# owensgroup/sparsify.me

Hardware: AMD Instinct MI355X
Metric: effective GF/s (2:4 spmma vs dense gemm) on ResNet-50 layer shapes (higher is better)
Workload: dtype f16

## Files before the change

### sparsify.me_amd/csrc/spmma_f16_fused.hip

```cpp
#include "select24.h"
#include "spmma_args.h"

namespace sm {

constexpr int MAXG = 8;
struct FusedArgs {
  const half_t* A[MAXG];
  const half_t* B[MAXG];
  half_t* C[MAXG];
  size_t sA, sB, sC;
  int Mrows, N, K, lda;
  int batch, tiles_m, tiles_n;
  int ngroup;
  float alpha, beta;
  const half_t* const* dAp;
  const half_t* const* dBp;
  half_t* const* dCp;
};

struct FusedArgsEpi : FusedArgs {
  EpiArgs e;
};
template <bool EPI> struct FusedArgsSel { typedef FusedArgs type; };
template <> struct FusedArgsSel<true> { typedef FusedArgsEpi type; };

template <int BN, int NS, bool BF = false, int BM = 128, int NWV = 4, bool ANT = true, bool DENSE = false, bool EPI = false>
__global__ __launch_bounds__(64 * NWV, (BN == 128 && NWV == 4 && BM == 128) ? 4 : 1) void spmma_f16_fused_direct_kernel(const typename FusedArgsSel<EPI>::type p) {
  static_assert(BM == 128 || BM == 64, "row tile");
  static_assert(NWV == 4 || (NWV == 8 && BM == 128), "waves per workgroup");
  constexpr int NW = NWV, TM = BM / NW, FM = TM / 16, FN = BN / 16;
  constexpr int SA = BM * 128, SB = 64 * BN * 2, STAGE = SA + SB;
  constexpr int A_N = BM / 8, B_N = BN / 8, W = A_N + B_N;
  static_assert(W % NW == 0, "equal DMA share per wave");
  constexpr int SL = W / NW;
  extern __shared__ __attribute__((aligned(16))) char smem[];

  const unsigned tid = threadIdx.x, lane = tid & 63u;
  const unsigned wave = __builtin_amdgcn_readfirstlane(tid >> 6);
  const unsigned tiles = (unsigned)p.tiles_m * (unsigned)p.tiles_n;
  const unsigned lid = tile_order(blockIdx.x, gridDim.x, true);
  const unsigned gb = lid / tiles, trem = lid - gb * tiles;
  const unsigned grp = gb / (unsigned)p.batch, b = gb - grp * (unsigned)p.batch;
  const unsigned tile_m = trem / (unsigned)p.tiles_n, tile_n = trem - tile_m * (unsigned)p.tiles_n;
  const int m0 = (int)tile_m * BM, n0 = (int)tile_n * BN;
  const int nkt = p.K / 64;
  const half_t* A = p.dAp ? p.dAp[gb] : p.A[grp] + (size_t)b * p.sA;
  const half_t* B = p.dBp ? p.dBp[gb] : p.B[grp] + (size_t)b * p.sB;
  half_t* C = p.dCp ? p.dCp[gb] : p.C[grp] + (size_t)b * p.sC;
  const int mlast = p.Mrows - 1;
  EpiBias<FM, FN> eb;
  if constexpr (EPI) eb = epi_bias_prefetch<FM, FN>(p.e, true, wave * TM, 0, m0, n0, p.Mrows, p.N, lane);

  const char* src[SL];
  size_t step[SL];
  unsigned loff[SL];
#pragma unroll
  for (int i = 0; i < SL; ++i) {
    const unsigned t = wave + (unsigned)NW * i;
    if (t < (unsigned)A_N) {
      const unsigned row = 8u * t + (lane >> 3), cs = (lane & 7u) ^ (row & 7u);
      int gr = m0 + (int)row;
      gr = gr < mlast ? gr : mlast;
      src[i] = reinterpret_cast<const char*>(A + (size_t)gr * p.lda) + 16u * cs;
      step[i] = 128;
      loff[i] = t * 1024u;
    } else {
      const unsigned j = t - A_N, panel = j >> 3, kr = 8u * (j & 7u) + (lane >> 3);
      const unsigned cs = (lane & 7u) ^ b_swz(kr);
      int gc = n0 + (int)(64u * panel + 8u * cs);
      gc = gc <= p.N - 8 ? gc : p.N - 8;
      src[i] = reinterpret_cast<const char*>(B + (size_t)kr * p.N + gc);
      step[i] = (size_t)64 * p.N * 2;
      loff[i] = SA + panel * 8192u + (j & 7u) * 1024u;
    }
  }
  auto stage = [&](int kt, int buf) {
    char* base = smem + buf * STAGE;
    static_assert(A_N % NW == 0, "A / B split of the DMA instructions is per instruction index");
#pragma unroll
    for (int i = 0; i < SL; ++i) {
      if (ANT && NW * i < A_N)
        __builtin_amdgcn_global_load_lds((gptr_t*)(src[i] + (size_t)kt * step[i]), (lptr_t*)(base + loff[i]), 16, 0, 2);
      else
        __builtin_amdgcn_global_load_lds((gptr_t*)(src[i] + (size_t)kt * step[i]), (lptr_t*)(base + loff[i]), 16, 0, 0);
    }
  };

  f4 acc[FM][FN];
#pragma unroll
  for (int i = 0; i < FM; ++i)
#pragma unroll
    for (int j = 0; j < FN; ++j) acc[i][j] = f4{0.f, 0.f, 0.f, 0.f};

#pragma unroll
  for (int s = 0; s < NS - 1; ++s)
    if (s < nkt) stage(s, s);
  int cur = 0, fill = NS - 1;
  for (int kt = 0; kt < nkt; ++kt) {
    const int ahead = (nkt - 1 - kt) < (NS - 2) ? (nkt - 1 - kt) : (NS - 2);
    if (NS >= 4 && ahead == 2) wait_dma_and_barrier<2 * SL>();
    else if (NS >= 3 && ahead == 1) wait_dma_and_barrier<SL>();
    else wait_dma_and_barrier<0>();
    if (kt + NS - 1 < nkt) stage(kt + NS - 1, fill);
    const char* As = smem + cur * STAGE;
    if constexpr (DENSE) mfma_stage_dense_a<FM, FN, BF>(As, As + SA, wave * TM, 0, lane, acc);
    else smfmac_stage_dense_a<FM, FN, BF>(As, As + SA, wave * TM, 0, lane, acc);
    cur = cur + 1 == NS ? 0 : cur + 1;
    fill = fill + 1 == NS ? 0 : fill + 1;
  }
  __syncthreads();
  if constexpr (EPI) store_c_tile_epi<BM, BN, FM, FN, 64 * NW, BF>(smem, C, p.e.R + (size_t)b * p.e.sR, p.e, eb, acc, true, wave * TM, 0, m0, n0, p.Mrows, p.N, p.alpha, p.beta, tid);
  else store_c_tile<BM, BN, FM, FN, 64 * NW, BF>(smem, C, acc, true, wave * TM, 0, m0, n0, p.Mrows, p.N, p.alpha, p.beta, tid);
}

template <int BN, int NS, bool BF = false, int BM = 128, int NWV = 4, bool ANT = true, bool DENSE = false, bool EPI = false>
static int launch_fused_direct(const typename FusedArgsSel<EPI>::type& a0, hipStream_t st) {
  typename FusedArgsSel<EPI>::type a = a0;
  a.tiles_m = (a.Mrows + BM - 1) / BM;
  a.tiles_n = (a.N + BN - 1) / BN;
  const size_t nwg = (size_t)a.tiles_m * a.tiles_n * a.batch * a.ngroup;
  constexpr size_t stage_bytes = BM * 128 + 64 * BN * 2;
  const size_t lds_main = ((size_t)(a.K / 64) < (size_t)NS ? (size_t)(a.K / 64) : (size_t)NS) * stage_bytes;
  constexpr size_t lds_epi = (size_t)BM * (BN * 2 + 16);
  const size_t lds = lds_main > lds_epi ? lds_main : lds_epi;
  constexpr size_t lds_max = NS * stage_bytes > lds_epi ? NS * stage_bytes : lds_epi;
  return launch_grid<&spmma_f16_fused_direct_kernel<BN, NS, BF, BM, NWV, ANT, DENSE, EPI>>(nwg, 64 * NWV, lds_max, lds, st, "sm_spmma_fused_f16",
                                                                                          "spmma_f16_fused_direct_kernel", a);
}

template <int BN, bool BF = false, int NSA = 3, int NSB = 2, bool ANT = true, bool DENSE = false, bool EPI = false>
__global__ __launch_bounds__(512) void spmma_f16_fused_big_kernel(const typename FusedArgsSel<EPI>::type p) {
  constexpr int BM = 256, NW = 8, TM = BM / NW, FM = TM / 16, FN = BN / 16;
  constexpr int SA = BM * 128, SB = 64 * BN * 2;
  constexpr int A_N = BM / 8, B_N = BN / 8;
  static_assert(A_N % NW == 0 && B_N % NW == 0, "equal DMA share per wave");
  static_assert(NSA == 3 && (NSB == 2 || NSB == 3), "ring depths the counted waits below are written for");
  constexpr int SLA = A_N / NW, SLB = B_N / NW;
  constexpr int AHEAD = SLA + (NSB == 3 ? SLB : 0);
  constexpr int BRING = NSA * SA;
  extern __shared__ __attribute__((aligned(16))) char smem[];

  const unsigned tid = threadIdx.x, lane = tid & 63u;
  const unsigned wave = __builtin_amdgcn_readfirstlane(tid >> 6);
  const unsigned tiles = (unsigned)p.tiles_m * (unsigned)p.tiles_n;
  const unsigned lid = xcd_remap(blockIdx.x, gridDim.x);
  const unsigned gb = lid / tiles, trem = lid - gb * tiles;
  const unsigned grp = gb / (unsigned)p.batch, b = gb - grp * (unsigned)p.batch;
  const unsigned tile_m = trem / (unsigned)p.tiles_n, tile_n = trem - tile_m * (unsigned)p.tiles_n;
  const int m0 = (int)tile_m * BM, n0 = (int)tile_n * BN;
  const int nkt = p.K / 64;
  const half_t* A = p.dAp ? p.dAp[gb] : p.A[grp] + (size_t)b * p.sA;
  const half_t* B = p.dBp ? p.dBp[gb] : p.B[grp] + (size_t)b * p.sB;
  half_t* C = p.dCp ? p.dCp[gb] : p.C[grp] + (size_t)b * p.sC;
  const int mlast = p.Mrows - 1;
// ... 370 lines not shown
    set_error("%s", why);
    return SM_STATUS_NOT_SUPPORTED;
  }
  SkPlan pl = sk_plan(panels, nkt, (size_t)a.tiles_n, (size_t)cus);
  const size_t nwg = (size_t)pl.slots * a.tiles_n;
  if (!workspace || !aligned16(workspace) || workspace_bytes < sk_workspace_bytes(nwg, BN)) {
    set_error("sm_spmma_fused_*_ws: the stream-K form needs a 16-byte aligned workspace of sm_spmma_fused_workspace_size bytes");
    return SM_STATUS_INVALID_VALUE;
  }
  SkArgs s = {};
  s.flags = reinterpret_cast<unsigned*>(workspace);
  s.part = reinterpret_cast<float*>(reinterpret_cast<char*>(workspace) + 4096);
  s.panels = (unsigned)panels; s.slots = pl.slots; s.tg = pl.tg; s.wg = pl.wg; s.groups_full = pl.groups_full; s.tgl = pl.tgl; s.wgl = pl.wgl;
  for (int i = 0; i < 9; ++i) { s.cut[i] = pl.cut[i]; s.cutl[i] = pl.cutl[i]; }
  constexpr size_t lds_main = (size_t)3 * BM * 128 + (size_t)2 * 64 * BN * 2;
  constexpr size_t lds_epi = (size_t)BM * (BN * 2 + 16);
  constexpr size_t lds = lds_main > lds_epi ? lds_main : lds_epi;
  static_assert(lds > 64 * 1024 && lds <= 160 * 1024, "LDS budget of the stream-K kernel (always opted in)");
  return launch_grid<&spmma_f16_fused_sk_kernel<BN, BF, ANT, DENSE>>(nwg, 512, lds, lds, st, "sm_spmma_fused_f16", "spmma_f16_fused_sk_kernel", a, s);
}

static bool sk_takes(size_t rows, size_t problems, size_t n, size_t k, bool astat_shape, size_t cus, SkPlan& pl) {
  if (n <= 128 || k < 128 || k % 64 != 0) return false;
  const size_t nkt = k / 64;
  const size_t panels = (rows + 255) / 256 * problems, tn = (n + 255) / 256;
  const size_t t_big = panels * tn, t_wide = (rows + 127) / 128 * tn * problems;
  pl = sk_plan(panels, nkt, tn, cus);
  if (!pl.slots) return false;
  const double c_sk = (double)pl.units + (pl.wg > 1 ? 8.0 : 0.0);
  const double c_big = (double)((t_big + cus - 1) / cus * nkt), c_wide = 0.6 * (double)((t_wide + cus - 1) / cus * nkt);
  const double c_now = c_big < c_wide ? c_big : c_wide;
  return !astat_shape && pl.wg > 1 && c_sk < 0.85 * c_now;
}

__device__ __attribute__((aligned(256))) const unsigned char sm_fused_zero_page[256] = {0};

template <int BN, bool BF = false, bool DENSE = false, bool EPI = false>
__global__ __launch_bounds__(256) void spmma_f16_fused_span_kernel(const typename FusedArgsSel<EPI>::type p, const unsigned span_lds ,
                                                                   const size_t a_bytes ) {
  constexpr int BM = 128, NW = 4, TM = BM / NW, FM = TM / 16, FN = BN / 16;
  constexpr int SB = 64 * BN * 2;
  extern __shared__ __attribute__((aligned(16))) char smem[];
  const unsigned tid = threadIdx.x, lane = tid & 63u;
  const unsigned wave = __builtin_amdgcn_readfirstlane(tid >> 6);
  const unsigned tiles = (unsigned)p.tiles_m * (unsigned)p.tiles_n;
  const unsigned lid = xcd_remap(blockIdx.x, gridDim.x);
  const unsigned grp = lid / tiles, trem = lid - grp * tiles;
  const unsigned tile_m = trem / (unsigned)p.tiles_n, tile_n = trem - tile_m * (unsigned)p.tiles_n;
  const int m0 = (int)tile_m * BM, n0 = (int)tile_n * BN;
  const int nkt = (p.K + 63) / 64;
  const char* A = reinterpret_cast<const char*>(p.dAp ? p.dAp[grp] : p.A[grp]);
  const half_t* B = p.dBp ? p.dBp[grp] : p.B[grp];
  half_t* C = p.dCp ? p.dCp[grp] : p.C[grp];
  const unsigned rowbytes = (unsigned)p.K * 2u;
  const int rows = p.Mrows - m0 < BM ? p.Mrows - m0 : BM;
  EpiBias<FM, FN> eb;
  if constexpr (EPI) eb = epi_bias_prefetch<FM, FN>(p.e, true, wave * TM, 0, m0, n0, p.Mrows, p.N, lane);

  {
    const size_t s0 = (size_t)m0 * rowbytes;
    const unsigned len = (unsigned)rows * rowbytes;
    const unsigned np = (len + 1023u) / 1024u;
    const size_t last16 = a_bytes - 16;
    for (unsigned pc = wave; pc < np; pc += NW) {
      size_t off = s0 + (size_t)pc * 1024u + 16u * lane;
      off = off < last16 ? off : last16;
      __builtin_amdgcn_global_load_lds((gptr_t*)(A + off), (lptr_t*)(smem + pc * 1024u), 16, 0, 2);
    }
  }
  char* const Bimg = smem + span_lds;
  {
    constexpr int B_N = BN / 8;
    const int npb = nkt * B_N;
    for (int t = (int)wave; t < npb; t += NW) {
      const int kt = t / B_N, j = t - kt * B_N;
      const unsigned panel = (unsigned)j >> 3, kr = 8u * ((unsigned)j & 7u) + (lane >> 3);
      const unsigned cs = (lane & 7u) ^ b_swz(kr);
      int gc = n0 + (int)(64u * panel + 8u * cs);
      gc = gc <= p.N - 8 ? gc : p.N - 8;
      const int krow = kt * 64 + (int)kr;
      const char* src = krow < p.K ? reinterpret_cast<const char*>(B + (size_t)krow * p.N + gc)
                                   : reinterpret_cast<const char*>(sm_fused_zero_page) + 16u * (lane & 7u);
      __builtin_amdgcn_global_load_lds((gptr_t*)src, (lptr_t*)(Bimg + kt * SB + panel * 8192u + ((unsigned)j & 7u) * 1024u), 16, 0, 0);
    }
  }
  wait_dma_and_barrier<0>();

  f4 acc[FM][FN];
#pragma unroll
  for (int i = 0; i < FM; ++i)
#pragma unroll
    for (int j = 0; j < FN; ++j) acc[i][j] = f4{0.f, 0.f, 0.f, 0.f};
  const unsigned g = lane >> 4, r = lane & 15u;
  unsigned rowoff[FM];
#pragma unroll
  for (int i = 0; i < FM; ++i) {
    int row = (int)(wave * TM + i * 16 + r);
    row = row < rows ? row : rows - 1;
    rowoff[i] = (unsigned)row * rowbytes;
  }
  for (int kt = 0; kt < nkt; ++kt) {
    if constexpr (DENSE) {
      h8 a0[FM], a1[FM];
#pragma unroll
      for (int i = 0; i < FM; ++i) {
        uint32_t d[2][4];
#pragma unroll
        for (int h = 0; h < 2; ++h) {
          const int k0 = kt * 64 + 32 * h + 8 * (int)g;
          int nv = p.K - k0;
          nv = nv < 0 ? 0 : (nv > 8 ? 8 : nv);
          const char* src = smem + rowoff[i] + 2u * (unsigned)k0;
#pragma unroll
          for (int e = 0; e < 4; ++e) {
            const uint32_t lo16 = *reinterpret_cast<const unsigned short*>(src + 4 * e);
            const uint32_t hi16 = *reinterpret_cast<const unsigned short*>(src + 4 * e + 2);
            uint32_t v = lo16 | (hi16 << 16);
            v = 2 * e + 1 < nv ? v : (2 * e < nv ? (v & 0xffffu) : 0u);
            d[h][e] = v;
          }
        }
        a0[i] = __builtin_bit_cast(h8, u4{d[0][0], d[0][1], d[0][2], d[0][3]});
        a1[i] = __builtin_bit_cast(h8, u4{d[1][0], d[1][1], d[1][2], d[1][3]});
      }
      mfma_b_sweep<FM, FN, BF>(a0, a1, Bimg + kt * SB, 0, lane, acc);
      continue;
    }
    h8 af[FM];
    int idx[FM];
    const int k0 = kt * 64 + 16 * (int)g;
    int nv = p.K - k0;
    nv = nv < 0 ? 0 : (nv > 16 ? 16 : nv);
#pragma unroll
    for (int i = 0; i < FM; ++i) {
      const char* src = smem + rowoff[i] + 2u * (unsigned)k0;
      uint32_t d[8];
#pragma unroll
      for (int e = 0; e < 8; ++e) {
        const uint32_t lo16 = *reinterpret_cast<const unsigned short*>(src + 4 * e);
        const uint32_t hi16 = *reinterpret_cast<const unsigned short*>(src + 4 * e + 2);
        uint32_t v = lo16 | (hi16 << 16);
        v = 2 * e + 1 < nv ? v : (2 * e < nv ? (v & 0xffffu) : 0u);
        d[e] = v;
      }
      dense16_to_operand(u4{d[0], d[1], d[2], d[3]}, u4{d[4], d[5], d[6], d[7]}, af[i], idx[i]);
    }
    smfmac_b_sweep<FM, FN, BF>(af, idx, Bimg + kt * SB, 0, lane, acc);
  }
  __syncthreads();
  if constexpr (EPI) store_c_tile_epi<BM, BN, FM, FN, 64 * NW, BF>(smem, C, p.e.R, p.e, eb, acc, true, wave * TM, 0, m0, n0, p.Mrows, p.N, p.alpha, p.beta, tid);
  else store_c_tile<BM, BN, FM, FN, 64 * NW, BF>(smem, C, acc, true, wave * TM, 0, m0, n0, p.Mrows, p.N, p.alpha, p.beta, tid);
}

template <int BN, bool BF = false, bool DENSE = false, bool EPI = false>
static int launch_fused_span(const typename FusedArgsSel<EPI>::type& a0, hipStream_t st) {
  typename FusedArgsSel<EPI>::type a = a0;
  a.tiles_m = (a.Mrows + 127) / 128;
  a.tiles_n = (a.N + BN - 1) / BN;
  const size_t nwg = (size_t)a.tiles_m * a.tiles_n * a.ngroup;
  if (nwg == 0) return SM_STATUS_SUCCESS;
  const size_t kc = ((size_t)a.K + 63) / 64 * 64;
  const size_t span_lds = ((size_t)128 * a.K * 2 + 128 + 1023) / 1024 * 1024;
  const size_t lds_main = span_lds + kc * BN * 2;
  constexpr size_t lds_epi = (size_t)128 * (BN * 2 + 16);
  const size_t lds = lds_main > lds_epi ? lds_main : lds_epi;
  if (lds > 160 * 1024 || nwg > 0x7fffffffu) {
    set_error("sm_spmma_fused_{f16,bf16}: k too long for the span form (use the staged path)");
    return SM_STATUS_NOT_SUPPORTED;
  }
  return launch_grid<&spmma_f16_fused_span_kernel<BN, BF, DENSE, EPI>>(nwg, 256, 160 * 1024, lds, st, "sm_spmma_fused_f16", "spmma_f16_fused_span_kernel", a,
                                                                      (unsigned)span_lds, (size_t)a.Mrows * a.K * 2);
}

template <int BN, int NBW>
struct BTileDma {
  static constexpr int B_WI = (BN / 8) / NBW;
  const char* src[B_WI];
  unsigned dst[B_WI];
  size_t step;
  __device__ __forceinline__ void setup(const half_t* B, int N, int n0, unsigned bw, unsigned lane, unsigned ring_off) {
#pragma unroll
    for (int i = 0; i < B_WI; ++i) {
      const unsigned j = bw + (unsigned)NBW * i, panel = j >> 3, grp = j & 7u, kr = 8u * grp + (lane >> 3);
      const unsigned cs = (lane & 7u) ^ b_swz(kr);
      int gc = n0 + (int)(64u * panel + 8u * cs);
      gc = gc <= N - 8 ? gc : N - 8;
      src[i] = reinterpret_cast<const char*>(B) + ((size_t)kr * N + (size_t)gc) * 2;
      dst[i] = ring_off + panel * 8192u + grp * 1024u;
    }
    step = (size_t)64 * N * 2;
  }
  __device__ __forceinline__ void issue(char* smem, int kt, unsigned buf_off) const {
#pragma unroll
    for (int i = 0; i < B_WI; ++i)
      __builtin_amdgcn_global_load_lds((gptr_t*)(src[i] + (size_t)kt * step), (lptr_t*)(smem + buf_off + dst[i]), 16, 0, 0);
  }
};


template <int BN, int WM, int WN, int NLB, int PF, int NSB, bool BF = false, bool ANT = true, bool EPI = false>
__global__ __launch_bounds__(64 * (WM * WN + 4 + NLB)) void spmma_f16_fused_wide_kernel(const typename FusedArgsSel<EPI>::type p) {
  constexpr int BM = 128, NLA = 4, NC = WM * WN, NW = NC + NLA + NLB;
  static_assert(PF >= 1 && PF <= 3 && NSB >= 2 && NSB <= 4, "pipeline depths");
  constexpr int TM = BM / WM, TN = BN / WN, FM = TM / 16, FN = TN / 16;
  constexpr int SA = BM * 64, SM_ = BM * 8, ASTG = SA + SM_, SB = 64 * BN * 2;
  constexpr int BRING = 2 * ASTG;
  constexpr int NBW = NLB > 0 ? NLB : WM * WN;
  constexpr int B_N = BN / 8, B_WI = B_N / NBW;
  static_assert(B_N % NBW == 0 && B_WI >= 1 && (NSB - 2) * B_WI <= 63, "B tile vs issuing waves");
  extern __shared__ __attribute__((aligned(16))) char smem[];

  const unsigned tid = threadIdx.x, lane = tid & 63u;
  const unsigned wave = __builtin_amdgcn_readfirstlane(tid >> 6);
  const unsigned tiles = (unsigned)p.tiles_m * (unsigned)p.tiles_n;
  const unsigned lid = xcd_remap(blockIdx.x, gridDim.x);
  const unsigned gb = lid / tiles, trem = lid - gb * tiles;
  const unsigned grp = gb / (unsigned)p.batch, b = gb - grp * (unsigned)p.batch;
  const unsigned tile_m = trem / (unsigned)p.tiles_n, tile_n = trem - tile_m * (unsigned)p.tiles_n;
  const int m0 = (int)tile_m * BM, n0 = (int)tile_n * BN;
  const int nkt = p.K / 64;
  half_t* C = p.C[grp] + (size_t)b * p.sC;

  f4 acc[FM][FN];
#pragma unroll
  for (int i = 0; i < FM; ++i)
#pragma unroll
    for (int j = 0; j < FN; ++j) acc[i][j] = f4{0.f, 0.f, 0.f, 0.f};
  const unsigned wm = wave / WN, wn = wave % WN;
  EpiBias<FM, FN> eb;
  if constexpr (EPI) eb = epi_bias_prefetch<FM, FN>(p.e, wave < (unsigned)NC, wm * TM, wn * TN, m0, n0, p.Mrows, p.N, lane);

  if (NLB > 0 && wave >= (unsigned)(NC + NLA)) {
    BTileDma<BN, NBW> bd;
    bd.setup(p.B[grp] + (size_t)b * p.sB, p.N, n0, wave - (NC + NLA), lane, BRING);
    auto issue = [&](int kt, int buf) {
      bd.issue(smem, kt, (unsigned)(buf * SB));
    };
#pragma unroll
    for (int s = 0; s < NSB - 1; ++s)
      if (s < nkt) issue(s, s);
    int nb = NSB - 1;
    for (int kt = 0; kt < nkt; ++kt) {
      if (kt + NSB - 2 < nkt) wait_dma_and_barrier<(NSB - 2) * B_WI>();
      else wait_dma_and_barrier<0>();
      if (kt + NSB - 1 < nkt) {
        issue(kt + NSB - 1, nb);
        nb = nb + 1 == NSB ? 0 : nb + 1;
      }
    }
  } else if (wave >= (unsigned)NC) {
    const unsigned lw = wave - NC;
    const half_t* A = p.A[grp] + (size_t)b * p.sA;
    const int mlast = p.Mrows - 1;
    const unsigned c8 = lane & 7u;
    const half_t* a_src[4];
    unsigned a_val_off[4], a_meta_off[4];
#pragma unroll
    for (int i = 0; i < 4; ++i) {
      const unsigned row = 8u * (4u * lw + i) + (lane >> 3);
      int gr = m0 + (int)row;
      gr = gr < mlast ? gr : mlast;
      a_src[i] = A + (size_t)gr * p.lda + 8u * c8;
      a_val_off[i] = row * 64u + 16u * ((c8 >> 1) ^ a64_swz(row)) + 8u * (c8 & 1u);
      a_meta_off[i] = SA + row * 8u + c8;
    }
    u4 ra[PF][4];
    auto load_a = [&](int kt, u4 (&dst)[4]) {
#pragma unroll
      for (int i = 0; i < 4; ++i) {
        if constexpr (ANT) dst[i] = __builtin_nontemporal_load(reinterpret_cast<const u4*>(a_src[i] + (size_t)kt * 64));
        else dst[i] = *reinterpret_cast<const u4*>(a_src[i] + (size_t)kt * 64);
      }
      __builtin_amdgcn_sched_barrier(0);
    };
    auto write_stage = [&](int kt, const u4 (&src)[4]) {
      char* sb = smem + (kt & 1) * ASTG;
#pragma unroll
      for (int i = 0; i < 4; ++i) {
        uint32_t k0, k1, n0, n1;
        strip_select_f16(src[i][0], src[i][1], k0, n0);
        strip_select_f16(src[i][2], src[i][3], k1, n1);
        *reinterpret_cast<u2*>(sb + a_val_off[i]) = u2{k0, k1};
        *reinterpret_cast<unsigned char*>(sb + a_meta_off[i]) = (unsigned char)(n0 | (n1 << 4));
      }
    };
    auto step = [&](int kt, u4 (&rr)[4], bool write, bool load) {
      asm volatile("s_waitcnt lgkmcnt(0)\n\ts_barrier" ::: "memory");
      __builtin_amdgcn_sched_barrier(0);
      if (write) {
        write_stage(kt + 1, rr);
      }
      if (load) load_a(kt + 1 + PF, rr);
      __builtin_amdgcn_sched_barrier(0);
    };
    int kt0 = 0;
    if (nkt > 2 * PF) {
#pragma unroll
      for (int s = 0; s < PF; ++s) load_a(s, ra[s]);
      write_stage(0, ra[0]);
      load_a(PF, ra[0]);
      for (; kt0 + 2 * PF < nkt; kt0 += PF) {
#pragma unroll
        for (int u = 0; u < PF; ++u) step(kt0 + u, ra[(u + 1) % PF], true, true);
      }
    } else {
#pragma unroll
      for (int s = 0; s < PF; ++s)
        if (s < nkt) load_a(s, ra[s]);
      write_stage(0, ra[0]);
      if (PF < nkt) load_a(PF, ra[0]);
    }
    for (; kt0 < nkt; kt0 += PF) {
#pragma unroll
// ... 408 lines not shown
    char* const patch = Cpatch + wave * WPATCH;
    f4 acc[FM][FN];
#pragma unroll
    for (int i = 0; i < FM; ++i)
#pragma unroll
      for (int j = 0; j < FN; ++j) acc[i][j] = f4{0.f, 0.f, 0.f, 0.f};
    int cb = 0, kt = 0, nt = nt0;
    for (int it = 0; it < T; ++it) {
      asm volatile("s_barrier" ::: "memory");
      const char* As = smem + kt * ASTG;
      const char* Ms = As + SA;
      const char* Bs = Bring + cb * SB;
      smfmac_stage<FM, FN, BF>(As, Ms, Bs, wm * TM, wn * TN, lane, acc);
      cb = cb + 1 == NSB ? 0 : cb + 1;
      if (++kt == nkt) {
        if constexpr (PR == TM) {
          const int gc = nt * BN + (int)(wn * TN) + 8 * (int)(lane & 7u);
#pragma unroll
          for (int i = 0; i < FM; ++i)
#pragma unroll
            for (int j = 0; j < FN; ++j) {
              const unsigned lr = i * 16 + 4u * g, lc = j * 16 + r;
#pragma unroll
              for (int q = 0; q < 4; ++q) {
                *reinterpret_cast<half_t*>(patch + (lr + q) * WPITCH + lc * 2) = to_elt<BF>(p.alpha * acc[i][j][q]);
                acc[i][j][q] = 0.f;
              }
            }
          asm volatile("s_waitcnt lgkmcnt(0)" ::: "memory");
#pragma unroll
          for (int s = 0; s < TM / 8; ++s) {
            const unsigned lr = 8u * s + (lane >> 3);
            const int gr = m0 + (int)(wm * TM + lr);
            if (gr < p.Mrows && gc < p.N) {
              const u2 lo = *reinterpret_cast<const u2*>(patch + lr * WPITCH + 16u * (lane & 7u));
              const u2 hi = *reinterpret_cast<const u2*>(patch + lr * WPITCH + 16u * (lane & 7u) + 8u);
              __builtin_nontemporal_store(u4{lo[0], lo[1], hi[0], hi[1]}, reinterpret_cast<u4*>(C + (size_t)gr * p.N + gc));
            }
          }
        } else {
          unsigned le = lane;
          asm volatile("" : "+v"(le));
          const int gce = nt * BN + (int)(wn * TN) + 8 * (int)(le & 7u);
#pragma unroll
          for (int i = 0; i < FM; ++i)
#pragma unroll
            for (int h = 0; h < 16 / PR; ++h) {
              if (PR == 16 || (g >> 1) == (unsigned)h) {
#pragma unroll
                for (int j = 0; j < FN; ++j) {
                  const unsigned lr = 4u * (g & (unsigned)(PR / 4 - 1)), lc = j * 16 + r;
#pragma unroll
                  for (int q = 0; q < 4; ++q) *reinterpret_cast<half_t*>(patch + (lr + q) * WPITCH + lc * 2) = to_elt<BF>(p.alpha * acc[i][j][q]);
                }
              }
              asm volatile("s_waitcnt lgkmcnt(0)" ::: "memory");
#pragma unroll
              for (int s = 0; s < PR / 8; ++s) {
                const unsigned lr = 8u * s + (le >> 3);
                const int gr = m0 + (int)(wm * TM + i * 16 + h * PR + lr);
                if (gr < p.Mrows && gce < p.N) {
                  const u2 lo = *reinterpret_cast<const u2*>(patch + lr * WPITCH + 16u * (le & 7u));
                  const u2 hi = *reinterpret_cast<const u2*>(patch + lr * WPITCH + 16u * (le & 7u) + 8u);
                  __builtin_nontemporal_store(u4{lo[0], lo[1], hi[0], hi[1]}, reinterpret_cast<u4*>(C + (size_t)gr * p.N + gce));
                }
              }
            }
#pragma unroll
          for (int i = 0; i < FM; ++i)
#pragma unroll
            for (int j = 0; j < FN; ++j) acc[i][j] = f4{0.f, 0.f, 0.f, 0.f};
        }
        kt = 0;
        ++nt;
      }
    }
  }
}


static size_t astat_nsplit(size_t panels, size_t tiles_n, size_t cus) {
  size_t nsplit = 1;
  while (panels * nsplit * 4 < 3 * cus && (tiles_n + 2 * nsplit - 1) / (2 * nsplit) >= 2) nsplit *= 2;
  return nsplit;
}
static size_t astat_lds_bytes(int nkt, int nsb) { return (size_t)nkt * (128 * 72) + (size_t)nsb * 64 * 128 * 2 + 8 * 32 * (64 * 2 + 8); }

constexpr int ASTAT_PAIR_NLB = 4;
static bool astat_pair_takes(int nkt, size_t nwg, int nsplit, size_t cus) { return nkt <= 3 || (nkt == 4 && nsplit == 1 && 4 * nwg >= 7 * cus); }
static size_t astat_pair_lds_bytes(int nkt) { return (size_t)nkt * (128 * 72) + (size_t)2 * 64 * 128 * 2 + 8 * (nkt <= 3 ? 16 : 8) * (64 * 2 + 8); }
static_assert(3 * (128 * 72) + 2 * 64 * 128 * 2 + 8 * 16 * 136 == 77824 && 4 * (128 * 72) + 2 * 64 * 128 * 2 + 8 * 8 * 136 == 78336, "LDS of the two-per-CU kernels");

template <auto KERNEL>
static bool two_resident_per_cu(unsigned threads, size_t lds, hipStream_t st) {
  static std::atomic<signed char> known[256];
  int dev = 0;
  if (hipGetDevice(&dev) != hipSuccess || dev < 0 || dev >= 256) return false;
  signed char k = known[dev].load(std::memory_order_relaxed);
  if (k == 0) {
    hipStreamCaptureStatus cs = hipStreamCaptureStatusNone;
    if (hipStreamIsCapturing(st, &cs) != hipSuccess) {
      (void)hipGetLastError();
      return false;
    }
    if (cs != hipStreamCaptureStatusNone) return false;
    static LdsOptIn optin;
    int nb = 0;
    if (ensure_dyn_lds(optin, reinterpret_cast<const void*>(KERNEL), lds, "spmma_f16_fused_astat_kernel") != SM_STATUS_SUCCESS ||
        hipOccupancyMaxActiveBlocksPerMultiprocessor(&nb, KERNEL, (int)threads, lds) != hipSuccess) {
      (void)hipGetLastError();
      nb = 0;
    }
    k = nb >= 2 ? 1 : -1;
    known[dev].store(k, std::memory_order_relaxed);
  }
  return k > 0;
}

template <bool BF = false>
static int launch_fused_astat(const FusedArgs& a0, hipStream_t st) {
  FusedArgs a = a0;
  a.tiles_m = (a.Mrows + 127) / 128;
  a.tiles_n = (a.N + 127) / 128;
  const size_t panels = (size_t)a.tiles_m * a.batch * a.ngroup;
  const size_t cus = (size_t)device_cu_count();
  int nsplit = (int)astat_nsplit(panels, (size_t)a.tiles_n, cus);
  int tps = (a.tiles_n + nsplit - 1) / nsplit;
  nsplit = (a.tiles_n + tps - 1) / tps;
  const size_t nwg = panels * nsplit;
  const int nkt = a.K / 64;
  if (astat_pair_takes(nkt, nwg, nsplit, cus)) {
    constexpr unsigned threads = 64 * (8 + ASTAT_PAIR_NLB);
    const size_t lds = astat_pair_lds_bytes(nkt);
    if (nkt <= 3) {
      constexpr auto kernel = &spmma_f16_fused_astat_kernel<2, BF, 0, ASTAT_PAIR_NLB, 16>;
      if (two_resident_per_cu<kernel>(threads, 80 * 1024, st))
        return launch_grid<kernel>(nwg, threads, 80 * 1024, lds, st, "sm_spmma_fused_f16", "spmma_f16_fused_astat_kernel", a, nsplit, tps);
    } else {
      constexpr auto kernel = &spmma_f16_fused_astat_kernel<2, BF, 0, ASTAT_PAIR_NLB, 8>;
      if (two_resident_per_cu<kernel>(threads, 80 * 1024, st))
        return launch_grid<kernel>(nwg, threads, 80 * 1024, lds, st, "sm_spmma_fused_f16", "spmma_f16_fused_astat_kernel", a, nsplit, tps);
    }
  }
  constexpr int NSB = 3;
  return launch_grid<&spmma_f16_fused_astat_kernel<NSB, BF>>(nwg, 64 * 16, 160 * 1024, astat_lds_bytes(a.K / 64, NSB), st, "sm_spmma_fused_f16",
                                                            "spmma_f16_fused_astat_kernel", a, nsplit, tps);
}

}

using namespace sm;

static bool span_lds_fits(size_t n, size_t k) { return ((size_t)128 * k * 2 + 1152) + ((k + 63) / 64 * 64) * (n <= 64 ? 64 : 128) * 2 <= 160 * 1024; }
static bool span_form_takes(size_t m, size_t n, size_t k, size_t lda, size_t batch, size_t strideA, size_t strideB, size_t strideC, bool all_aligned, bool c_aligned) {
  return (k % 64 != 0 || lda % 8 != 0) && lda == k && n % 8 == 0 && n <= 128 && all_aligned && c_aligned && (batch == 1 || (strideB == 0 && strideA == m * lda && strideC == m * n)) &&
         (m * batch * k * 2) % 16 == 0 && m * batch <= 0x7fffffffull && k <= 0x7fffffffull && span_lds_fits(n, k);
}
static bool stage_forms_take(size_t n, size_t k, size_t lda, size_t strideA, size_t strideB, bool all_aligned) {
  return !(k % 64 != 0 || lda % 8 != 0 || strideA % 8 != 0 || n % 8 != 0 || strideB % 8 != 0 || !all_aligned);
}
static bool dims_fit_int(size_t m, size_t n, size_t k, size_t lda, size_t batch) {
  return !(m * batch > 0x7fffffffull || n > 0x7fffffffull || k > 0x7fffffffull || lda > 0x7fffffffull);
}

struct FusedCall {
  size_t m, n, k, lda, batch, count, sA, sB, sC;
  float beta;
  bool a_aligned, b_aligned, c_aligned;
  bool ws, ws_aligned;
  size_t ws_bytes;
  bool epi, r_aligned;
  size_t sR;
};
struct FusedPick {
  int form;
  bool stacked;
  const char* why;
};

static FusedPick fused_form(const FusedCall& c, size_t cus) {
  const size_t m = c.m, n = c.n, k = c.k, lda = c.lda, batch = c.batch;
  if (c.count == 0 || m == 0 || n == 0 || batch == 0) return {SM_FUSED_FORM_EMPTY, false, nullptr};
  const bool all_aligned = c.a_aligned && c.b_aligned;
  const bool contiguous = c.sB == 0 && c.sA == m * lda && c.sC == m * n;
  if (n < 8 && k <= 64 && lda == k && (batch == 1 || contiguous)) {
    if (c.epi) return {SM_FUSED_FORM_NOT_TAKEN, false, "sm_spmma_fused_{f16,bf16}_ex: the thin form (n < 8) takes no epilogue"};
    if (thin_form_takes(c.count, m * batch, n, k) && c.a_aligned) return {SM_FUSED_FORM_THIN, true, nullptr};
  }
  const bool r_follows = !c.epi || c.beta == 0.0f || (c.r_aligned && (batch == 1 || c.sR == m * n));
  if (span_form_takes(m, n, k, lda, batch, c.sA, c.sB, c.sC, all_aligned, c.c_aligned && r_follows)) return {SM_FUSED_FORM_SPAN, true, nullptr};
  if (!stage_forms_take(n, k, lda, c.sA, c.sB, all_aligned))
    return {SM_FUSED_FORM_NOT_TAKEN, false, "sm_spmma_fused_{f16,bf16}: needs k % 64 == 0, n % 8 == 0 and 16-byte aligned rows (use the staged path)"};
  if (c.count > 1 && !c.c_aligned)
    return {SM_FUSED_FORM_NOT_TAKEN, false, "sm_spmma_fused_{f16,bf16}_grouped: needs 16-byte aligned C operands"};
  if (!dims_fit_int(m, n, k, lda, batch)) return {SM_FUSED_FORM_NOT_TAKEN, false, "sm_spmma_fused_{f16,bf16}: dimension exceeds 2^31-1"};
  const bool stacked = batch > 1 && contiguous && (!c.epi || c.beta == 0.0f || c.sR == m * n);
  const size_t rows = stacked ? m * batch : m, nb = (stacked ? 1 : batch) * c.count;
  const bool astat_store = n > 256 && k <= 512 && c.beta == 0.0f && c.c_aligned && (c.sC % 8 == 0);
  if (c.ws) {
    SkPlan pl;
    if (sk_takes(rows, nb, n, k, astat_store, cus, pl) && c.ws_bytes >= sk_workspace_bytes((size_t)pl.slots * ((n + 255) / 256), 256) && c.ws_aligned &&
        !sk_launch_limits((rows + 255) / 256 * nb, n, k, lda, cus))
      return {SM_FUSED_FORM_STREAMK, stacked, nullptr};
  }
  auto round_eff = [](size_t tiles, size_t cus_) { const size_t r = (tiles + cus_ - 1) / cus_; return r ? (double)tiles / (double)(r * cus_) : 1.0; };
  if (n > 128 && k > 64) {
    const size_t t_big = (rows + 255) / 256 * ((n + 255) / 256) * nb, t_wide = (rows + 127) / 128 * ((n + 255) / 256) * nb;
    bool big = round_eff(t_big, cus) >= round_eff(t_wide, cus);
    if (!c.epi && astat_store) {
      const size_t panels = (rows + 127) / 128 * nb;
      big = round_eff(t_big, cus) > round_eff(panels * astat_nsplit(panels, (n + 127) / 128, cus), cus) + 0.1;
    }
    if (big) return {SM_FUSED_FORM_BIG, stacked, nullptr};
  }
  if (n <= 128 || (n <= 256 && k <= 64)) {
    if (n <= 64) return {SM_FUSED_FORM_DIRECT64, stacked, nullptr};
    return {n > 128 || k < 512 ? SM_FUSED_FORM_DIRECT128 : SM_FUSED_FORM_DIRECT128_NT, stacked, nullptr};
  }
  if (!c.epi && astat_store && astat_lds_bytes((int)(k / 64), 3) <= 160 * 1024) return {SM_FUSED_FORM_ASTAT, stacked, nullptr};
  if (k <= 1024 && !c.epi) return {SM_FUSED_FORM_WIDEP, stacked, nullptr};
  return {n > 256 ? SM_FUSED_FORM_WIDE : SM_FUSED_FORM_WIDE_NT, stacked, nullptr};
}

static bool fused_form_is_exact(int form) { return form != SM_FUSED_FORM_NOT_TAKEN && form != SM_FUSED_FORM_EMPTY && form != SM_FUSED_FORM_THIN; }

bool sm::spmma_fused16_takes_exact(const void* A, const void* B, const void* C, size_t m, size_t n, size_t k, size_t lda, size_t batch, size_t strideA, size_t strideB,
                                   size_t strideC) {
  if (!A || !B || !C || lda < k) return false;
  const FusedCall c = {m, n, k, lda, batch, 1, strideA, strideB, strideC, 0.0f, aligned16(A), aligned16(B), aligned16(C), false, false, 0, false, false, 0};
  return fused_form_is_exact(fused_form(c, 256).form);
}

extern "C" int sm_spmma_fused_form(size_t m, size_t n, size_t k, size_t lda, size_t batch, size_t count, size_t strideA, size_t strideB, size_t strideC,
                                   float beta, unsigned flags, size_t cus, int* form) {
  constexpr unsigned known = SM_FUSED_FLAG_A_ALIGNED | SM_FUSED_FLAG_B_ALIGNED | SM_FUSED_FLAG_C_ALIGNED | SM_FUSED_FLAG_WORKSPACE | SM_FUSED_FLAG_EPILOGUE;
  if (!form || lda < k || count > (size_t)MAXG || (flags & ~known) || ((flags & SM_FUSED_FLAG_WORKSPACE) && (flags & SM_FUSED_FLAG_EPILOGUE))) {
    set_error("sm_spmma_fused_form: invalid argument");
    return SM_STATUS_INVALID_VALUE;
  }
  const bool c_al = (flags & SM_FUSED_FLAG_C_ALIGNED) != 0, ws = (flags & SM_FUSED_FLAG_WORKSPACE) != 0;
  const FusedCall c = {m, n, k, lda, batch, count, strideA, strideB, strideC, beta, (flags & SM_FUSED_FLAG_A_ALIGNED) != 0, (flags & SM_FUSED_FLAG_B_ALIGNED) != 0, c_al,
                       ws, ws, ws ? ~(size_t)0 : 0, (flags & SM_FUSED_FLAG_EPILOGUE) != 0, c_al, strideC};
  *form = fused_form(c, cus ? cus : (size_t)device_cu_count()).form;
  return SM_STATUS_SUCCESS;
}

template <bool BF>
static int spmma_fused16(size_t ngroup, const void* const* Ag, const void* const* Bg, void* const* Cg, size_t m, size_t n, size_t k, size_t lda,
                         size_t batch, size_t strideA, size_t strideB, size_t strideC, float alpha, float beta,
                         sm_stream_t stream, void* workspace = nullptr, size_t workspace_bytes = 0, const EpiArgs* epi = nullptr) {
#define SM_LAUNCH(fn, ...) (epi ? fn<__VA_ARGS__, true>(ae, st) : fn<__VA_ARGS__, false>(a, st))
  if (ngroup == 0) return SM_STATUS_SUCCESS;
  if (!Ag || !Bg || !Cg || lda < k || ngroup > (size_t)MAXG) {
    set_error("sm_spmma_fused_{f16,bf16}: invalid argument");
    return SM_STATUS_INVALID_VALUE;
  }
  FusedCall c = {m, n, k, lda, batch, ngroup, strideA, strideB, strideC, beta, true, true, true, workspace != nullptr, aligned16(workspace), workspace_bytes,
                 epi != nullptr, epi && aligned16(epi->R), epi ? epi->sR : 0};
  for (size_t g = 0; g < ngroup; ++g) {
    if (!Ag[g] || !Bg[g] || !Cg[g]) {
      set_error("sm_spmma_fused_{f16,bf16}: invalid argument (null operand)");
      return SM_STATUS_INVALID_VALUE;
    }
    c.a_aligned = c.a_aligned && aligned16(Ag[g]);
    c.b_aligned = c.b_aligned && aligned16(Bg[g]);
    c.c_aligned = c.c_aligned && aligned16(Cg[g]);
  }
  const FusedPick pick = fused_form(c, (size_t)device_cu_count());
  hipStream_t st = (hipStream_t)stream;
  FusedArgs a = {};
  for (size_t g = 0; g < (size_t)MAXG; ++g) {
    const size_t s_ = g < ngroup ? g : 0;
    a.A[g] = (const half_t*)Ag[s_]; a.B[g] = (const half_t*)Bg[s_]; a.C[g] = (half_t*)Cg[s_];
  }
  a.ngroup = (int)ngroup;
  a.N = (int)n; a.K = (int)k; a.lda = (int)lda;
  a.alpha = alpha; a.beta = beta;
  if (pick.stacked) {
    a.Mrows = (int)(m * batch);
    a.batch = 1;
  } else {
    a.Mrows = (int)m;
    a.batch = (int)batch;
  }
  if (pick.form != SM_FUSED_FORM_SPAN) { a.sA = strideA; a.sB = strideB; a.sC = strideC; }
  FusedArgsEpi ae = {};
  static_cast<FusedArgs&>(ae) = a;
  if (epi) ae.e = *epi;
  switch (pick.form) {
    case SM_FUSED_FORM_EMPTY: return SM_STATUS_SUCCESS;
    case SM_FUSED_FORM_NOT_TAKEN:
      set_error("%s", pick.why);
      return SM_STATUS_NOT_SUPPORTED;
    case SM_FUSED_FORM_THIN: return spmma_fused_thin(BF, (int)ngroup, Ag, Bg, Cg, m * batch, n, k, alpha, beta, st);
    case SM_FUSED_FORM_SPAN: return n <= 64 ? SM_LAUNCH(launch_fused_span, 64, BF, false) : SM_LAUNCH(launch_fused_span, 128, BF, false);
    case SM_FUSED_FORM_STREAMK:
      return n <= 256 ? launch_fused_sk<256, BF, true>(a, workspace, workspace_bytes, st) : launch_fused_sk<256, BF, false>(a, workspace, workspace_bytes, st);
    case SM_FUSED_FORM_BIG: return n <= 256 ? SM_LAUNCH(launch_fused_big, 256, BF, 3, 2, true, false) : SM_LAUNCH(launch_fused_big, 256, BF, 3, 2, false, false);
    case SM_FUSED_FORM_DIRECT64: return SM_LAUNCH(launch_fused_direct, 64, 2, BF, 128, 4, true, false);
    case SM_FUSED_FORM_DIRECT128: return SM_LAUNCH(launch_fused_direct, 128, 2, BF, 128, 4, false, false);
    case SM_FUSED_FORM_DIRECT128_NT: return SM_LAUNCH(launch_fused_direct, 128, 2, BF, 128, 4, true, false);
    case SM_FUSED_FORM_ASTAT: return launch_fused_astat<BF>(a, st);
    case SM_FUSED_FORM_WIDEP: return launch_fused_widep<256, 4, 2, 4, 2, 3, BF>(a, st);
    case SM_FUSED_FORM_WIDE: return SM_LAUNCH(launch_fused_wide, 256, 4, 2, 4, 2, 3, BF, false);
    case SM_FUSED_FORM_WIDE_NT: return SM_LAUNCH(launch_fused_wide, 256, 4, 2, 4, 2, 3, BF, true);
  }
// ... 151 lines not shown
```

Baseline: 594,700.

## Add streaming span kernel with per-wave A ring buffer for short-K shapes

Adds a new span-form kernel in which each of 12 waves owns a small LDS ring of 16-row A blocks. The ring is filled with asynchronous global-to-LDS loads tracked by vmcnt waits, while B is staged once per workgroup and reused across every block that workgroup handles. Work is split into per-CU chunks of 16-row blocks instead of 128-row tiles, and C is written through an LDS patch using nontemporal stores. It targets odd-K layers such as the K=147 stem conv, where the old span kernel needed 128·K of LDS per tile and had low parallelism. The cost is hand-written waitcnt sequencing and single-fragment MFMA use per wave, which may lower arithmetic density.

```diff
diff --git a/sparsify.me_amd/csrc/spmma_f16_fused.hip b/sparsify.me_amd/csrc/spmma_f16_fused.hip
--- a/sparsify.me_amd/csrc/spmma_f16_fused.hip
+++ b/sparsify.me_amd/csrc/spmma_f16_fused.hip
@@ -1,5 +1,7 @@
 #include "select24.h"
 #include "spmma_args.h"
+
+static bool span_stream_takes(size_t n, size_t k);
 
 namespace sm {
 
@@ -676,6 +678,152 @@
   else store_c_tile<BM, BN, FM, FN, 64 * NW, BF>(smem, C, acc, true, wave * TM, 0, m0, n0, p.Mrows, p.N, p.alpha, p.beta, tid);
 }
 
+constexpr int SPAN_STREAM_NW = 12;
+constexpr int SPAN_STREAM_R = 2;
+constexpr int SPAN_STREAM_MAX_WAIT = 23;
+
+__device__ __forceinline__ void wait_vmcnt_upto(unsigned n) {
+#define SM_WAIT_CASE(N) case N: asm volatile("s_waitcnt vmcnt(" #N ")" ::: "memory"); break;
+  switch (n) {
+    SM_WAIT_CASE(1) SM_WAIT_CASE(2) SM_WAIT_CASE(3) SM_WAIT_CASE(4) SM_WAIT_CASE(5) SM_WAIT_CASE(6) SM_WAIT_CASE(7) SM_WAIT_CASE(8)
+    SM_WAIT_CASE(9) SM_WAIT_CASE(10) SM_WAIT_CASE(11) SM_WAIT_CASE(12) SM_WAIT_CASE(13) SM_WAIT_CASE(14) SM_WAIT_CASE(15) SM_WAIT_CASE(16)
+    SM_WAIT_CASE(17) SM_WAIT_CASE(18) SM_WAIT_CASE(19) SM_WAIT_CASE(20) SM_WAIT_CASE(21) SM_WAIT_CASE(22) SM_WAIT_CASE(23)
+    default: asm volatile("s_waitcnt vmcnt(0)" ::: "memory"); break;
+  }
+#undef SM_WAIT_CASE
+}
+static_assert(SPAN_STREAM_MAX_WAIT == 23 && SPAN_STREAM_MAX_WAIT < 64, "wait_vmcnt_upto's cases; vmcnt is 6 bits");
+
+template <int BN, bool BF = false, int NW = SPAN_STREAM_NW, int R = SPAN_STREAM_R>
+__global__ __launch_bounds__(64 * NW) void spmma_f16_fused_span_stream_kernel(const FusedArgs p, const unsigned slot ,
+                                                                              const size_t a_bytes ,
+                                                                              const unsigned wg_per_problem, const unsigned blocks_per_wg) {
+  constexpr int FN = BN / 16, SB = 64 * BN * 2, CPITCH = BN * 2 + 16;
+  constexpr int NST = 16 * (BN / 8) / 64;
+  static_assert(R >= 2 && (R - 1) * NST < SPAN_STREAM_MAX_WAIT, "ring");
+  extern __shared__ __attribute__((aligned(16))) char smem[];
+  const unsigned tid = threadIdx.x, lane = tid & 63u;
+  const unsigned wave = __builtin_amdgcn_readfirstlane(tid >> 6);
+  const unsigned grp = blockIdx.x / wg_per_problem, wgi = blockIdx.x - grp * wg_per_problem;
+  const int nkt = (p.K + 63) / 64;
+  const char* A = reinterpret_cast<const char*>(p.A[grp]);
+  const half_t* B = p.B[grp];
+  half_t* C = p.C[grp];
+  const unsigned rowbytes = (unsigned)p.K * 2u;
+  const unsigned blkbytes = 16u * rowbytes;
+  const unsigned np = (blkbytes + 1023u) / 1024u;
+  const unsigned nblocks = ((unsigned)p.Mrows + 15u) / 16u;
+  const unsigned first = wgi * blocks_per_wg + wave;
+  const unsigned end = (wgi + 1u) * blocks_per_wg < nblocks ? (wgi + 1u) * blocks_per_wg : nblocks;
+  const unsigned cnt = first < end ? (end - first + (unsigned)NW - 1u) / (unsigned)NW : 0u;
+
+  {
+    constexpr int B_N = BN / 8;
+    const int npb = nkt * B_N;
+    for (int t = (int)wave; t < npb; t += NW) {
+      const int kt = t / B_N, j = t - kt * B_N;
+      const unsigned panel = (unsigned)j >> 3, kr = 8u * ((unsigned)j & 7u) + (lane >> 3);
+      const unsigned cs = (lane & 7u) ^ b_swz(kr);
+      int gc = (int)(64u * panel + 8u * cs);
+      gc = gc <= p.N - 8 ? gc : p.N - 8;
+      const int krow = kt * 64 + (int)kr;
+      const char* src = krow < p.K ? reinterpret_cast<const char*>(B + (size_t)krow * p.N + gc)
+                                   : reinterpret_cast<const char*>(sm_fused_zero_page) + 16u * (lane & 7u);
+      __builtin_amdgcn_global_load_lds((gptr_t*)src, (lptr_t*)(smem + kt * SB + panel * 8192u + ((unsigned)j & 7u) * 1024u), 16, 0, 0);
+    }
+  }
+  char* const ring = smem + nkt * SB + wave * (unsigned)R * slot;
+  const unsigned ring_addr = (unsigned)(uintptr_t)(lds_char*)ring;
+  const size_t last16 = a_bytes - 16;
+  auto issue = [&](unsigned i) {
+    const size_t s0 = (size_t)(first + i * (unsigned)NW) * blkbytes + 16u * lane;
+    char* dst = ring + (i % (unsigned)R) * slot;
+    for (unsigned pc = 0; pc < np; ++pc) {
+      size_t off = s0 + (size_t)pc * 1024u;
+      off = off < last16 ? off : last16;
+      __builtin_amdgcn_global_load_lds((gptr_t*)(A + off), (lptr_t*)(dst + pc * 1024u), 16, 0, 2);
+    }
+  };
+  unsigned pre = cnt < (unsigned)(R - 1) ? cnt : (unsigned)(R - 1);
+  for (unsigned i = 0; i < pre; ++i) issue(i);
+  wait_vmcnt_upto(pre * np);
+  __builtin_amdgcn_s_barrier();
+
+  const unsigned g = lane >> 4, r = lane & 15u;
+  for (unsigned i = 0; i < cnt; ++i) {
+    const unsigned blk = first + i * (unsigned)NW;
+    const unsigned as_addr = ring_addr + (i % (unsigned)R) * slot;
+    if (i + (unsigned)(R - 1) < cnt) issue(i + (unsigned)(R - 1));
+    {
+      const unsigned ahead = cnt - 1u - i < (unsigned)(R - 1) ? cnt - 1u - i : (unsigned)(R - 1);
+      const unsigned stored = i < (unsigned)(R - 1) ? i : (unsigned)(R - 1);
+      wait_vmcnt_upto(ahead * np + stored * (unsigned)NST);
+    }
+    const int rows = p.Mrows - (int)(blk * 16u) < 16 ? p.Mrows - (int)(blk * 16u) : 16;
+    const unsigned row = (int)r < rows ? r : (unsigned)(rows - 1);
+    const unsigned rowoff = row * rowbytes;
+    f4 acc[1][FN];
+#pragma unroll
+    for (int j = 0; j < FN; ++j) acc[0][j] = f4{0.f, 0.f, 0.f, 0.f};
+    for (int kt = 0; kt < nkt; ++kt) {
+      h8 af[1];
+      int idx[1];
+      const int k0 = kt * 64 + 16 * (int)g;
+      int nv = p.K - k0;
+      nv = nv < 0 ? 0 : (nv > 16 ? 16 : nv);
+      u4 lo, hi;
+      asm volatile("ds_read_b128 %0, %2\n\tds_read_b128 %1, %2 offset:16\n\ts_waitcnt lgkmcnt(0)"
+                   : "=&v"(lo), "=&v"(hi) : "v"(as_addr + rowoff + 2u * (unsigned)k0) : "memory");
+      uint32_t d[8] = {lo[0], lo[1], lo[2], lo[3], hi[0], hi[1], hi[2], hi[3]};
+#pragma unroll
+      for (int e = 0; e < 8; ++e) d[e] = 2 * e + 1 < nv ? d[e] : (2 * e < nv ? (d[e] & 0xffffu) : 0u);
+      dense16_to_operand(u4{d[0], d[1], d[2], d[3]}, u4{d[4], d[5], d[6], d[7]}, af[0], idx[0]);
+      smfmac_b_sweep<1, FN, BF>(af, idx, smem + kt * SB, 0, lane, acc);
+    }
+    {
+      const unsigned wr = as_addr + 4u * g * CPITCH + 2u * r;
+#pragma unroll
+      for (int j = 0; j < FN; ++j)
+#pragma unroll
+        for (int q = 0; q < 4; ++q) {
+          const uint32_t v = __builtin_bit_cast(unsigned short, to_elt<BF>(p.alpha * acc[0][j][q]));
+          asm volatile("ds_write_b16 %0, %1" ::"v"(wr + (unsigned)(q * CPITCH + j * 32)), "v"(v) : "memory");
+        }
+    }
+    u4 cv[NST];
+#pragma unroll
+    for (int t = 0; t < NST; ++t) {
+      const unsigned q = lane + 64u * t, prow = q / (BN / 8), cn = q % (BN / 8);
+      asm volatile("ds_read_b128 %0, %1" : "=v"(cv[t]) : "v"(as_addr + prow * CPITCH + cn * 16u) : "memory");
+    }
+    asm volatile("s_waitcnt lgkmcnt(0)" ::: "memory");
+#pragma unroll
+    for (int t = 0; t < NST; ++t) {
+      const unsigned q = lane + 64u * t, prow = q / (BN / 8), cn = q % (BN / 8);
+      const int gr = (int)(blk * 16u + prow), gc = 8 * (int)cn;
+      if (gr < p.Mrows && gc < p.N)
+        __builtin_nontemporal_store(cv[t], reinterpret_cast<u4*>(C + (size_t)gr * p.N + gc));
+    }
+  }
+}
+
+constexpr size_t SPAN_STREAM_LDS_MAX = 160 * 1024;
+static constexpr size_t span_stream_slot_bytes(size_t k, size_t bn) {
+  const size_t blk = (16 * k * 2 + 160 + 1023) / 1024 * 1024, patch = (16 * (bn * 2 + 16) + 1023) / 1024 * 1024;
+  return blk > patch ? blk : patch;
+}
+static constexpr size_t span_stream_lds_bytes(size_t n, size_t k) {
+  const size_t bn = n <= 64 ? 64 : 128;
+  return (k + 63) / 64 * 64 * bn * 2 + (size_t)SPAN_STREAM_NW * SPAN_STREAM_R * span_stream_slot_bytes(k, bn);
+}
+static_assert(span_stream_lds_bytes(64, 147) == 24 * 1024 + 12 * 2 * 5 * 1024 && span_stream_lds_bytes(64, 147) <= SPAN_STREAM_LDS_MAX,
+              "k = 147, n = 64: 144 KiB");
+static size_t span_stream_blocks_per_wg(size_t nblocks, size_t problems, size_t cus) {
+  const size_t per = cus / problems ? cus / problems : 1;
+  const size_t even = (nblocks + per - 1) / per;
+  return even > 4 ? even : 4;
+}
+
 template <int BN, bool BF = false, bool DENSE = false, bool EPI = false>
 static int launch_fused_span(const typename FusedArgsSel<EPI>::type& a0, hipStream_t st) {
   typename FusedArgsSel<EPI>::type a = a0;
@@ -683,6 +831,17 @@
   a.tiles_n = (a.N + BN - 1) / BN;
   const size_t nwg = (size_t)a.tiles_m * a.tiles_n * a.ngroup;
   if (nwg == 0) return SM_STATUS_SUCCESS;
+  if constexpr (!DENSE && !EPI) {
+    constexpr auto kernel = &spmma_f16_fused_span_stream_kernel<BN, BF>;
+    if (a.beta == 0.0f && !a.dAp && span_stream_takes((size_t)a.N, (size_t)a.K)) {
+      const size_t nblocks = ((size_t)a.Mrows + 15) / 16;
+      const size_t bpw = span_stream_blocks_per_wg(nblocks, (size_t)a.ngroup, (size_t)device_cu_count());
+      const size_t wgp = (nblocks + bpw - 1) / bpw;
+      return launch_grid<kernel>(wgp * a.ngroup, 64 * SPAN_STREAM_NW, SPAN_STREAM_LDS_MAX, span_stream_lds_bytes((size_t)a.N, (size_t)a.K), st, "sm_spmma_fused_f16",
+                                 "spmma_f16_fused_span_stream_kernel", a, (unsigned)span_stream_slot_bytes((size_t)a.K, BN), (size_t)a.Mrows * a.K * 2,
+                                 (unsigned)wgp, (unsigned)bpw);
+    }
+  }
   const size_t kc = ((size_t)a.K + 63) / 64 * 64;
   const size_t span_lds = ((size_t)128 * a.K * 2 + 128 + 1023) / 1024 * 1024;
   const size_t lds_main = span_lds + kc * BN * 2;
@@ -1397,6 +1556,10 @@
 using namespace sm;
 
 static bool span_lds_fits(size_t n, size_t k) { return ((size_t)128 * k * 2 + 1152) + ((k + 63) / 64 * 64) * (n <= 64 ? 64 : 128) * 2 <= 160 * 1024; }
+static bool span_stream_takes(size_t n, size_t k) {
+  const size_t np = (16 * k * 2 + 1023) / 1024, nst = (n <= 64 ? 64 : 128) / 32;
+  return span_stream_lds_bytes(n, k) <= SPAN_STREAM_LDS_MAX && (SPAN_STREAM_R - 1) * (np + nst) <= (size_t)SPAN_STREAM_MAX_WAIT;
+}
 static bool span_form_takes(size_t m, size_t n, size_t k, size_t lda, size_t batch, size_t strideA, size_t strideB, size_t strideC, bool all_aligned, bool c_aligned) {
   return (k % 64 != 0 || lda % 8 != 0) && lda == k && n % 8 == 0 && n <= 128 && all_aligned && c_aligned && (batch == 1 || (strideB == 0 && strideA == m * lda && strideC == m * n)) &&
          (m * batch * k * 2) % 16 == 0 && m * batch <= 0x7fffffffull && k <= 0x7fffffffull && span_lds_fits(n, k);
```

Result: no change. 599,400 (median of 6 runs) (+0.8%).
